# 14chanwa/remotesensingProject

Measured on AMD Instinct MI355X. Metric: Mpixel*disparity-hypotheses/s, higher is better.
Workload: dtype f32

## Files before the change

remotesensingproject_amd/build.py:

```python
from __future__ import annotations

import os
import re
import subprocess
import sys

HERE = os.path.dirname(os.path.abspath(__file__))
CSRC = os.path.join(HERE, "csrc")
OBJ = os.path.join(CSRC, "build")
SO = os.path.join(CSRC, "librslf_hip.so")
INCLUDE = os.path.join(os.path.dirname(HERE), "include")
COMMON = ["rslf_internal.hpp", "rslf_plan.hpp", "rslf_scratch.hpp", "rslf_device.hpp", "k2_taps.hpp", os.path.join(INCLUDE, "rslf_hip.h")]
UNITS = {
    "rslf_core.hip": ["k0_pack.hpp"],
    "rslf_pile.hip": ["k1_edge.hpp", "k_compact.hpp", "k2_scan.hpp", "k2_reg.hpp", "k2_stream.hpp", "k3_median.hpp"],
    "rslf_chip_a.hip": ["k2_scan.hpp", "k2_chip.hpp"],
    "rslf_chip_b.hip": ["k2_scan.hpp", "k2_chip.hpp"],
    "rslf_chip_c.hip": ["k2_scan.hpp", "k2_chip.hpp"],
    "rslf_scores.hip": ["k2_scan.hpp", "k2_reg.hpp", "k2_scores.hpp"],
    "rslf_peaks.hip": ["k8_peaks.hpp", "k8_peak_rule.hpp", "rslf_plan_peaks.hpp"],
    "rslf_subgrid.hip": ["k2_scan.hpp", "k9_subgrid.hpp", "k8_peak_rule.hpp", "rslf_plan_subgrid.hpp"],
    "rslf_sweep.hip": ["k3_median.hpp", "k4_propagate.hpp", "k_compact.hpp", "k2_scan.hpp", "k7_line_conf.hpp", "rslf_plan_subgrid.hpp",
                       "rslf_plan_sweep_peaks.hpp", "rslf_plan_peaks.hpp", "rslf_plan_sweep_gate.hpp", "k11_f2c_peak_rule.hpp"],
    "rslf_sweep_peaks.hip": ["k2_scan.hpp", "k10_sweep_peaks.hpp", "k10_peak_merge.hpp", "k8_peak_rule.hpp", "rslf_plan_sweep_peaks.hpp",
                             "rslf_plan_peaks.hpp", "rslf_plan_subgrid.hpp"],
    "rslf_f2c.hip": ["k5_f2c.hpp", "rslf_plan_f2c_peaks.hpp", "rslf_plan_peaks.hpp", "rslf_plan_f2c_consistency.hpp",
                     "rslf_plan_consistency.hpp", "k12_consistency_rule.hpp"],
    "rslf_f2c_keep.hip": ["rslf_plan_f2c_peaks.hpp", "rslf_plan_peaks.hpp", "rslf_plan_sweep_gate.hpp", "k11_f2c_peak_rule.hpp",
                          "rslf_plan_f2c_consistency.hpp", "rslf_plan_consistency.hpp", "k12_consistency_rule.hpp"],
    "rslf_f2c_peaks.hip": ["k11_f2c_peaks.hpp", "k11_f2c_peak_rule.hpp", "rslf_plan_f2c_peaks.hpp", "rslf_plan_peaks.hpp"],
    "rslf_render.hip": ["k6_render.hpp", "rslf_plan_render.hpp"],
    "rslf_consistency.hip": ["k12_consistency.hpp", "k12_consistency_rule.hpp", "rslf_plan_consistency.hpp", "k13_f2c_consistency.hpp",
                             "rslf_plan_f2c_consistency.hpp"],
    "rslf_warp.hip": ["k14_view_warp.hpp", "k14_warp_rule.hpp", "rslf_plan_warp.hpp", "k12_consistency_rule.hpp"],
    "rslf_multi.hip": [],
    "rslf_multi_sweep.hip": [],
}
SOURCES = list(UNITS)

HIPCC_FLAGS = [
    "--offload-arch=gfx950",
    "-O3",
    "-std=c++17",
    "-fPIC",
    "-ffp-contract=off",
    "-fno-fast-math",
    "-fno-slp-vectorize",
]


def _hipcc() -> str:
    for c in (os.environ.get("HIPCC"), "/opt/rocm/bin/hipcc", "hipcc"):
        if c and (os.path.isabs(c) and os.path.exists(c) or not os.path.isabs(c)):
            return c
    raise RuntimeError("hipcc not found")


def _deps(unit: str) -> list[str]:
    out = []
    for d in [unit] + UNITS[unit] + COMMON:
        p = d if os.path.isabs(d) else os.path.join(CSRC, d)
        if os.path.exists(p):
            out.append(p)
    return out


def _obj(unit: str) -> str:
    return os.path.join(OBJ, unit.replace(".hip", ".o"))


def _stale(unit: str) -> bool:
    o = _obj(unit)
    return not os.path.exists(o) or any(os.path.getmtime(d) > os.path.getmtime(o) for d in _deps(unit))


def needs_build() -> bool:
    return not os.path.exists(SO) or any(_stale(u) or os.path.getmtime(_obj(u)) > os.path.getmtime(SO) for u in SOURCES)


def source_hash() -> str:
    import hashlib
    h = hashlib.sha256()
    files = sorted(set(p for u in SOURCES for p in _deps(u)))
    for p in files:
        h.update(os.path.basename(p).encode() + b"\0")
        h.update(open(p, "rb").read())
    return h.hexdigest()[:16]


def build_variant(name: str, defines: list[str]) -> str:
    import concurrent.futures
    out_dir = os.path.join(os.path.dirname(HERE), "ab")
    os.makedirs(out_dir, exist_ok=True)
    os.makedirs(OBJ, exist_ok=True)

    def compile_unit(u: str) -> str:
        obj = os.path.join(OBJ, "%s_%s.o" % (os.path.splitext(u)[0], name))
        r = subprocess.run([_hipcc()] + HIPCC_FLAGS + ["-D" + d for d in defines] + ["-I", INCLUDE, "-c", u, "-o", obj],
                           cwd=CSRC, capture_output=True, text=True)
        if r.returncode != 0:
            raise RuntimeError("hipcc failed on %s:\n%s" % (u, r.stderr[-4000:]))
        return obj

    with concurrent.futures.ThreadPoolExecutor(max_workers=min(len(SOURCES), os.cpu_count() or 1)) as ex:
        objs = list(ex.map(compile_unit, SOURCES))
    so = os.path.join(out_dir, "librslf_%s.so" % name)
# ... 66 lines not shown
```

remotesensingproject_amd/csrc/k4_propagate.hpp:

```cpp
#pragma once

#include "k_compact.hpp"
#include "k11_f2c_peak_rule.hpp"
#include "k3_median.hpp"
#include "rslf_device.hpp"

#ifndef RSLF_CLAIM_BATCH
#define RSLF_CLAIM_BATCH 8
#endif

namespace rslf {

constexpr int kClaimMaxViews = 1024;
constexpr int kNoWinner = 0x7F7F7F7F;

template <int C>
__device__ __forceinline__ void propagate_claim_pixel(const VolView& vol, int s_hat, int v, int u, float cur, bool source,
                                                      const float* __restrict__ rbar_vu, const uint8_t* __restrict__ mask_svu,
                                                      int* __restrict__ winner_svu, uint8_t* __restrict__ dirty, float slope,
                                                      const plan::NormThreshold& prop_thr, const unsigned long long* live_views)
{
    const int nseg = (vol.U + 255) >> 8;
    const long long o = (long long)v * vol.U + u;
    float rb[C];
#pragma unroll
    for (int c = 0; c < C; c++)
        rb[c] = source ? rbar_vu[o * C + c] : 0.0f;
    const long long plane = (long long)vol.V * vol.U;
    const long long row = (long long)v * vol.U;
    constexpr int B = RSLF_CLAIM_BATCH;
    for (int s0 = 0; s0 < vol.S; s0 += B) {
        int ri[B];
        bool live[B];
        static_assert(64 % B == 0, "a batch of views sits in one word of the live-view bits");
        if (live_views && ((live_views[s0 >> 6] >> (s0 & 63)) & ((1ull << B) - 1ull)) == 0)
            continue;
        uint8_t mb[B];
#pragma unroll
        for (int j = 0; j < B; j++) {
            const int s = s0 + j;
            float off = cur * (float)(s_hat - s);
            off = off * slope;
            ri[j] = u + (int)roundf(off);
            live[j] = source && s < vol.S && ri[j] >= 0 && ri[j] < vol.U;
            ri[j] = min(max(ri[j], 0), vol.U - 1);
            mb[j] = mask_svu[(long long)min(s, vol.S - 1) * plane + row + ri[j]];
        }
        bool any = false;
#pragma unroll
        for (int j = 0; j < B; j++) {
            live[j] = live[j] && mb[j] != 0;
            any |= live[j];
        }
        if (!__any(any))
            continue;
        float e[B][C];
#pragma unroll
        for (int j = 0; j < B; j++) {
            const float* er = vol.row(v, min(s0 + j, vol.S - 1));
            const int col = live[j] ? ri[j] : min(u, vol.U - 1);
#pragma unroll
            for (int c = 0; c < C; c++)
                e[j][c] = er[col * C + c];
        }
#pragma unroll
        for (int j = 0; j < B; j++) {
            if (!live[j])
                continue;
            float df[C];
#pragma unroll
            for (int c = 0; c < C; c++)
                df[c] = e[j][c] - rb[c];
            if (norm_below<C>(df, prop_thr)) {
                atomicMin(&winner_svu[(long long)(s0 + j) * plane + row + ri[j]], u);
                dirty[((long long)(s0 + j) * vol.V + v) * nseg + (ri[j] >> 8)] = 1;
            }
        }
    }
}

struct ClaimGate {
    const int32_t* idx;
    const float* score;
    const int32_t* runner_idx;
    const float* runner_score;
    long long hat;
    float ratio;
    unsigned long long* withheld;
// ... 93 lines not shown
                                                       uint8_t* __restrict__ dirty, float slope, plan::NormThreshold prop_thr,
                                                       const float* __restrict__ gate_Cd_vu, float disp_thr, int* __restrict__ reset,
                                                       const int* __restrict__ remain)
{
    median_claim_body<C, MODE, false>(vol, s_hat, raw_vu, filtered_vu, edge_mask_vu, w, median_thr, rbar_vu, mask_svu, winner_svu, dirty,
                                      slope, prop_thr, gate_Cd_vu, disp_thr, reset, remain, ClaimGate{});
}

template <int C, int MODE>
__global__ __launch_bounds__(256) void k34_median_claim_gated(VolView vol, int s_hat, const float* __restrict__ raw_vu,
                                                             float* __restrict__ filtered_vu, const uint8_t* __restrict__ edge_mask_vu,
                                                             int w, plan::NormThreshold median_thr, const float* __restrict__ rbar_vu,
                                                             const uint8_t* __restrict__ mask_svu, int* __restrict__ winner_svu,
                                                             uint8_t* __restrict__ dirty, float slope, plan::NormThreshold prop_thr,
                                                             const float* __restrict__ gate_Cd_vu, float disp_thr,
                                                             int* __restrict__ reset, const int* __restrict__ remain, ClaimGate gate)
{
    median_claim_body<C, MODE, true>(vol, s_hat, raw_vu, filtered_vu, edge_mask_vu, w, median_thr, rbar_vu, mask_svu, winner_svu, dirty,
                                     slope, prop_thr, gate_Cd_vu, disp_thr, reset, remain, gate);
}

struct ApplyPeaks {
    int32_t* idx;
    float* score;
    int32_t* runner_idx;
    float* runner_score;
};

template <bool PEAKS>
__device__ __forceinline__ void apply_segment(long long r, int seg, int V, int U, const float* __restrict__ filtered_vu,
                                              const float* __restrict__ Cd_hat_vu, float* __restrict__ depth_svu,
                                              float* __restrict__ Cd_svu, uint8_t* mask_svu, int* __restrict__ winner_svu,
                                              int* __restrict__ remain, const float* __restrict__ Cl_hat_vu,
                                              float* __restrict__ Cl_svu, const ApplyPeaks& pk, long long hat)
{
    const int u = (seg << 8) + threadIdx.x;
    const long long t = r * U + (u < U ? u : U - 1);
    const int w = u < U ? winner_svu[t] : U;
    const unsigned long long leaving = __ballot(w < U);
    if (remain && leaving && (threadIdx.x & 63) == 0)
        atomicSub(&remain[r * ((U + 255) >> 8) + seg], __popcll(leaving));
    if (w >= U)
        return;
    const long long src = (r % V) * U + w;
    depth_svu[t] = filtered_vu[src];
    Cd_svu[t] = Cd_hat_vu[src];
    if (Cl_svu)
        Cl_svu[t] = Cl_hat_vu[src];
    if (PEAKS) {
        if (pk.idx)
            pk.idx[t] = pk.idx[hat + src];
        if (pk.score)
            pk.score[t] = pk.score[hat + src];
        if (pk.runner_idx)
            pk.runner_idx[t] = pk.runner_idx[hat + src];
        if (pk.runner_score)
            pk.runner_score[t] = pk.runner_score[hat + src];
    }
    mask_svu[t] = 0;
    winner_svu[t] = kNoWinner;
}

__global__ __launch_bounds__(256) void k4_count_segments(const uint8_t* __restrict__ mask_svu, long long rows, int U, int* __restrict__ remain)
{
    const int nseg = (U + 255) >> 8;
    const long long item = blockIdx.x;
    if (item >= rows * nseg)
        return;
    const long long r = item / nseg;
    const int seg = (int)(item - r * nseg);
    const int u = (seg << 8) + threadIdx.x;
    const unsigned long long b = __ballot(u < U && mask_svu[r * U + (u < U ? u : 0)] != 0);
    __shared__ int s_n[4];
    if ((threadIdx.x & 63) == 0)
        s_n[threadIdx.x >> 6] = __popcll(b);
    __syncthreads();
    if (threadIdx.x == 0)
        remain[item] = s_n[0] + s_n[1] + s_n[2] + s_n[3];
}

constexpr int kApplyRowsPerBlock = 4;
constexpr int kApplyFlagSlots = 1024;

template <bool PEAKS>
__device__ __forceinline__ void propagate_apply_body(int S, int V, int U, int s_hat, const float* __restrict__ filtered_vu,
                                                         const float* __restrict__ Cd_hat_vu, float* __restrict__ depth_svu,
                                                         float* __restrict__ Cd_svu, uint8_t* mask_svu, int* __restrict__ winner_svu,
                                                         uint8_t* __restrict__ dirty, int s_next, const uint8_t* __restrict__ edge_mask_next_vu,
                                                         int* __restrict__ list, int* __restrict__ count,
                                                         unsigned long long* __restrict__ total, int* __restrict__ packed_n,
                                                         int* __restrict__ remain, int* __restrict__ rowbase,
                                                         const float* __restrict__ Cl_hat_vu, float* __restrict__ Cl_svu, const ApplyPeaks& pk)
{
    __shared__ uint8_t s_flags[kApplyFlagSlots];
    const long long hat = PEAKS ? (long long)s_hat * V * U : 0;
    const int nseg = (U + 255) >> 8;
    const int lead = s_next >= 0 ? V : 0;
    if ((int)blockIdx.x < lead) {
        const int v = blockIdx.x;
        const long long r = (long long)s_next * V + v;
        uint8_t* flags = dirty + r * nseg;
        for (int seg = 0; seg < nseg; seg++)
            if (flags[seg])
                apply_segment<PEAKS>(r, seg, V, U, filtered_vu, Cd_hat_vu, depth_svu, Cd_svu, mask_svu, winner_svu, remain, Cl_hat_vu, Cl_svu, pk, hat);
        __syncthreads();
        if ((int)threadIdx.x < nseg)
            flags[threadIdx.x] = 0;
        compact_row_packed(v, edge_mask_next_vu, mask_svu + (long long)s_next * V * U, U, list, count, total, packed_n, rowbase);
        return;
    }
    const long long nrows = (long long)S * V;
    const long long r0 = (long long)(blockIdx.x - lead) * kApplyRowsPerBlock;
    const long long r1 = r0 + kApplyRowsPerBlock < nrows ? r0 + kApplyRowsPerBlock : nrows;
    const int nfl = (int)(r1 - r0) * nseg;
    for (int i = threadIdx.x; i < nfl; i += 256) {
        const long long r = r0 + i / nseg;
        uint8_t f = 0;
        if ((int)(r / V) != s_next) {
            f = dirty[r0 * nseg + i];
            if (f)
                dirty[r0 * nseg + i] = 0;
        }
        s_flags[i] = f;
    }
    __syncthreads();
    for (int i = 0; i < nfl; i++)
        if (s_flags[i])
            apply_segment<PEAKS>(r0 + i / nseg, i % nseg, V, U, filtered_vu, Cd_hat_vu, depth_svu, Cd_svu, mask_svu, winner_svu, remain, Cl_hat_vu, Cl_svu, pk, hat);
}

__global__ __launch_bounds__(256) void k4_propagate_apply(int S, int V, int U, int s_hat, const float* __restrict__ filtered_vu,
                                                         const float* __restrict__ Cd_hat_vu, float* __restrict__ depth_svu,
                                                         float* __restrict__ Cd_svu, uint8_t* mask_svu, int* __restrict__ winner_svu,
                                                         uint8_t* __restrict__ dirty, int s_next, const uint8_t* __restrict__ edge_mask_next_vu,
                                                         int* __restrict__ list, int* __restrict__ count,
                                                         unsigned long long* __restrict__ total, int* __restrict__ packed_n,
                                                         int* __restrict__ remain, int* __restrict__ rowbase,
                                                         const float* __restrict__ Cl_hat_vu, float* __restrict__ Cl_svu)
{
    propagate_apply_body<false>(S, V, U, s_hat, filtered_vu, Cd_hat_vu, depth_svu, Cd_svu, mask_svu, winner_svu, dirty, s_next,
                                edge_mask_next_vu, list, count, total, packed_n, remain, rowbase, Cl_hat_vu, Cl_svu, ApplyPeaks{});
}

__global__ __launch_bounds__(256) void k4_propagate_apply_peaks(int S, int V, int U, int s_hat, const float* __restrict__ filtered_vu,
                                                               const float* __restrict__ Cd_hat_vu, float* __restrict__ depth_svu,
                                                               float* __restrict__ Cd_svu, uint8_t* mask_svu, int* __restrict__ winner_svu,
                                                               uint8_t* __restrict__ dirty, int s_next,
                                                               const uint8_t* __restrict__ edge_mask_next_vu, int* __restrict__ list,
                                                               int* __restrict__ count, unsigned long long* __restrict__ total,
                                                               int* __restrict__ packed_n, int* __restrict__ remain, int* __restrict__ rowbase,
                                                               const float* __restrict__ Cl_hat_vu, float* __restrict__ Cl_svu, ApplyPeaks pk)
{
    propagate_apply_body<true>(S, V, U, s_hat, filtered_vu, Cd_hat_vu, depth_svu, Cd_svu, mask_svu, winner_svu, dirty, s_next,
                               edge_mask_next_vu, list, count, total, packed_n, remain, rowbase, Cl_hat_vu, Cl_svu, pk);
}

}
```

remotesensingproject_amd/csrc/rslf_core.hip:

```cpp
#include "rslf_internal.hpp"

#include <algorithm>
#include <cmath>

#include "k0_pack.hpp"

using namespace rslf;


namespace rslf {

char* last_error_buffer()
{
    static thread_local char g_err[512] = "";
    return g_err;
}

static std::atomic<int> g_inject[kInjectSites];

bool inject_hit(InjectSite site)
{
    std::atomic<int>& c = g_inject[site];
    int v = c.load(std::memory_order_relaxed);
    while (v > 0)
// ... 138 lines not shown
{
    if (!out)
        return fail(RSLF_ERR_INVALID_ARG, "out is NULL");
    *out = nullptr;
    int n = 0;
    if (hipGetDeviceCount(&n) != hipSuccess || n <= 0)
        return fail(RSLF_ERR_NO_DEVICE, "no HIP device visible");
    if (device < 0 || device >= n)
        return fail(RSLF_ERR_INVALID_ARG, "device %d out of range (0..%d)", device, n - 1);
    hipDeviceProp_t prop;
    HIP_TRY(hipGetDeviceProperties(&prop, device));
    if (strncmp(prop.gcnArchName, "gfx950", 6) != 0)
        return fail(RSLF_ERR_NO_DEVICE, "device %d is %s; this library holds gfx950 code objects only", device, prop.gcnArchName);
    HIP_TRY(hipSetDevice(device));
    rslf_ctx* ctx = new (std::nothrow) rslf_ctx();
    if (!ctx)
        return fail(RSLF_ERR_ALLOC, "out of host memory");
    ctx->device = device;
    (void)hipDeviceGetAttribute(&ctx->num_cus, hipDeviceAttributeMultiprocessorCount, device);
    hipError_t e = hip_err(ctx->scratch.total.reserve(2 * sizeof(unsigned long long)));
    if (e == hipSuccess)
        e = hip_err(ctx->scratch.minmax.reserve(2 * sizeof(float)));
    if (e == hipSuccess)
        e = hipEventCreate(&ctx->ev0);
    if (e == hipSuccess)
        e = hipEventCreate(&ctx->ev1);
    if (e != hipSuccess) {
        (void)rslf_ctx_destroy(ctx);
        return fail(RSLF_ERR_HIP, "context setup failed: %s", hipGetErrorString(e));
    }
    *out = ctx;
    return RSLF_OK;
}
RSLF_API_CATCH

extern "C" int rslf_ctx_destroy(rslf_ctx* ctx) RSLF_API_TRY
{
    if (!ctx)
        return RSLF_OK;
    (void)hipSetDevice(ctx->device);
    (void)hipStreamSynchronize(ctx->stream);
    for (hipEvent_t e : ctx->ev_pool)
        (void)hipEventDestroy(e);
    if (ctx->ev0)
        (void)hipEventDestroy(ctx->ev0);
    if (ctx->ev1)
        (void)hipEventDestroy(ctx->ev1);
    delete ctx;
    return RSLF_OK;
}
RSLF_API_CATCH

extern "C" int rslf_ctx_set_stream(rslf_ctx* ctx, void* hip_stream) RSLF_API_TRY
{
    if (!ctx)
        return fail(RSLF_ERR_INVALID_ARG, "ctx is NULL");
    ctx->stream = (hipStream_t)hip_stream;
    return RSLF_OK;
}
RSLF_API_CATCH

extern "C" int rslf_ctx_set_debug(rslf_ctx* ctx, const char* key, int value) RSLF_API_TRY
{
    if (!ctx || !key)
        return fail(RSLF_ERR_INVALID_ARG, "ctx/key is NULL");
    if (strcmp(key, "force_scan") == 0 && value >= 0 && value <= 2)
        ctx->force_scan = value;
    else if (strcmp(key, "force_groups") == 0 && value >= 0 && value <= 64)
        ctx->force_groups = value;
    else if (strcmp(key, "force_packed") == 0 && value >= -1 && value <= 1)
        ctx->force_packed = value;
    else if (strcmp(key, "px") == 0 && value >= -1 && value <= 1)
        ctx->px_mode = value;
    else if (strcmp(key, "stream_share") == 0 && value >= 0 && value <= 2)
        ctx->stream_share = value;
    else if (strcmp(key, "row_split") == 0 && value >= 0 && value <= 65536)
        ctx->row_split = value;
    else if (strcmp(key, "tap_table") == 0 && (value == 0 || value == 1))
        ctx->tap_table = value;
    else if (strcmp(key, "scalar_taps") == 0 && (value == 0 || value == 1))
        ctx->scalar_taps = value;
    else if (strcmp(key, "claim_skip") == 0 && (value == 0 || value == 1))
        ctx->claim_skip = value;
    else if (strcmp(key, "subgrid_list") == 0 && (value == 0 || value == 1))
        ctx->subgrid_list = value;
    else if (strcmp(key, "peaks_list") == 0 && (value == 0 || value == 1))
        ctx->peaks_list = value;
    else if (strcmp(key, "consistency_order") == 0 && value >= 0 && value <= 2)
        ctx->consistency_order = value;
    else if (strcmp(key, "time_all") == 0 && (value == 0 || value == 1)) {
        ctx->time_all = value;
        ctx->ev_used = 0;
    } else if (strcmp(key, "stream_groups") == 0 && value >= 0 && value <= 64)
        ctx->stream_groups = value;
    else if (strcmp(key, "stream_lds_kib") == 0 && value >= 16 && value <= 152) {
        ctx->stream_lds_bytes = (size_t)value << 10;
    } else if (strcmp(key, "staging_kib") == 0 && value >= 0 && value <= 262144)
        ctx->staging_kib = value;
    else
        return fail(RSLF_ERR_INVALID_ARG, "rslf_ctx_set_debug: unknown key or value out of range: %s = %d", key, value);
    return RSLF_OK;
}
RSLF_API_CATCH

extern "C" int rslf_ctx_synchronize(rslf_ctx* ctx) RSLF_API_TRY
{
    if (!ctx)
        return fail(RSLF_ERR_INVALID_ARG, "ctx is NULL");
    HIP_TRY(hipSetDevice(ctx->device));
    HIP_TRY(hipStreamSynchronize(ctx->stream));
    return RSLF_OK;
}
RSLF_API_CATCH


extern "C" int rslf_volume_create(rslf_ctx* ctx, int V, int S, int U, int C, rslf_volume** out) RSLF_API_TRY
{
    if (!ctx || !out)
        return fail(RSLF_ERR_INVALID_ARG, "ctx/out is NULL");
    *out = nullptr;
    if (V < 1 || S < 1 || U < 1)
        return fail(RSLF_ERR_INVALID_ARG, "bad dimensions V=%d S=%d U=%d", V, S, U);
    if (C != 1 && C != 3)
        return fail(RSLF_ERR_UNSUPPORTED, "C=%d: the reference instantiates float and cv::Vec3f only (dc.hpp:149-154)", C);
    if (V > 65535 || S > 65535)
        return fail(RSLF_ERR_UNSUPPORTED, "V=%d / S=%d: the per-scanline kernels index scanlines and views with grid.y / grid.z "
                                          "(at most 65535)", V, S);
    if ((long long)S * C * (((long long)U + 1 + 63) / 64 * 64) > ((long long)1 << 29))
        return fail(RSLF_ERR_UNSUPPORTED, "one EPI (S*pitch*C floats) must stay below 2 GiB: the scan addresses it with 32-bit byte offsets");
    HIP_TRY(hipSetDevice(ctx->device));
    rslf_volume* vol = new (std::nothrow) rslf_volume();
    if (!vol)
        return fail(RSLF_ERR_ALLOC, "out of host memory");
    vol->ctx = ctx;
    vol->device = ctx->device;
    vol->V = V;
    vol->S = S;
    vol->U = U;
    vol->C = C;
    vol->pitch = plan::volume_pitch(U);
    vol->bytes = plan::volume_bytes(V, S, U, C);
    hipError_t e = hipMalloc(&vol->base, vol->bytes);
    if (e != hipSuccess) {
        delete vol;
        return fail(RSLF_ERR_ALLOC, "hipMalloc(%zu) for the volume failed: %s", vol->bytes, hipGetErrorString(e));
    }
    *out = vol;
    return RSLF_OK;
}
RSLF_API_CATCH

extern "C" int rslf_volume_destroy(rslf_volume* vol) RSLF_API_TRY
{
    if (!vol)
        return RSLF_OK;
    (void)hipSetDevice(vol->device);
    (void)hipFree(vol->base);
    delete vol;
    return RSLF_OK;
}
RSLF_API_CATCH

extern "C" int rslf_volume_describe(const rslf_volume* vol, rslf_volume_desc* out) RSLF_API_TRY
{
    if (!vol || !out)
        return fail(RSLF_ERR_INVALID_ARG, "vol/out is NULL");
// ... 428 lines not shown
```

remotesensingproject_amd/csrc/rslf_internal.hpp:

```cpp
#pragma once

#include "../../include/rslf_hip.h"

#include <hip/hip_runtime.h>

#include <atomic>
#include <cstdarg>
#include <cstdio>
#include <cstring>
#include <exception>
#include <functional>
#include <memory>
#include <new>
#include <string>
#include <thread>
#include <vector>

#include "rslf_device.hpp"
#include "rslf_plan.hpp"
#include "rslf_scratch.hpp"


namespace rslf {

// ... 146 lines not shown
    DeviceBuf withheld;
    DeviceBuf lc_columns;
    DeviceBuf lc_argmax;
    DeviceBuf shared[kSharedBufs];

    static constexpr size_t kMaxPartials = 2048;
    unsigned long long* pixel_total() const { return total.as<unsigned long long>(); }
    int* packed_len() const { return reinterpret_cast<int*>(pixel_total() + 1); }
    uint8_t* morph_tmp() const { return depth_tmp.as<uint8_t>(); }
};

constexpr int row_exact_slots(int spad, int C) { return (C == 1 && spad == 104) ? spad : 0; }
constexpr size_t row_exact_bytes(int dim_d, int slots) { return (size_t)dim_d * ((size_t)slots * 16 + 8); }

struct RowExactKey {
    float dmin = 0.0f, dmax = 0.0f, slope = 0.0f;
    int dim_d = 0, s_hat = 0, S = 0, U = 0, C = 0, slots = 0;
    long long stride_s = 0;
    const void* queued_on = nullptr;
    bool same(const RowExactKey& o) const
    {
        return memcmp(&dmin, &o.dmin, sizeof(float)) == 0 && memcmp(&dmax, &o.dmax, sizeof(float)) == 0 &&
               memcmp(&slope, &o.slope, sizeof(float)) == 0 && dim_d == o.dim_d && s_hat == o.s_hat && S == o.S && U == o.U && C == o.C &&
               slots == o.slots && stride_s == o.stride_s && queued_on == o.queued_on;
    }
};

struct SweepState {
    bool open = false;
    bool keep_total = false;
    bool first = true;
    bool scanned = false;
    bool listed = false;
    int expect = -1;
    uint8_t* mask_run = nullptr;
    int lc_mode = RSLF_LINE_CONF_OFF;
    float* lc_Cl_svu = nullptr;
    float* lc_K_vsu = nullptr;
    int32_t* lc_idx_vu = nullptr;
    const float* lc_Ce_svu = nullptr;
    const float* lc_dmin_vu = nullptr;
    const float* lc_dmax_vu = nullptr;
    float lc_dmin = 0.0f, lc_dmax = 0.0f;
    int lc_dim_d = 0;
    ScanConsts lc_consts = {};
    bool subgrid = false;
    bool peaks = false;
    rslf_peaks pk = {};
    int dim_d = 0;
    float prop_ratio = 0.0f;
};

}

struct rslf_ctx {
    int device = 0;
    hipStream_t stream = nullptr;
    rslf::Scratch scratch;
    rslf::SweepState sweep;
    hipEvent_t ev0 = nullptr, ev1 = nullptr;
    bool ev_valid = false;
    int time_all = 0;
    std::vector<hipEvent_t> ev_pool;
    size_t ev_used = 0;
    int last_spad = 0;
    int last_kernel = 0;
    bool last_gated = false;
    int num_cus = 0;
    int force_scan = 0;
    int force_groups = 0;
    int force_packed = -1;
    int px_mode = -1;
    int stream_groups = 0;
    int stream_share = 1;
    size_t stream_lds_bytes = rslf::plan::kStreamLdsBytes;
    int row_split = 1;
    int tap_table = 1;
    int scalar_taps = 1;
    rslf::RowExactKey row_exact_key;
    bool last_row_exact = false;
    int subgrid_list = 1;
    int peaks_list = 1;
    int claim_skip = 1;
    int staging_kib = 0;
    int consistency_order = 0;
};

struct rslf_volume {
    rslf_ctx* ctx = nullptr;
    int device = 0;
    int V = 0, S = 0, U = 0, C = 0, pitch = 0;
    float* base = nullptr;
    size_t bytes = 0;
    float min_value = 0.0f, max_value = 0.0f;
    bool filled = false;
};

struct rslf_multi {
    struct Dev {
        rslf_ctx* ctx = nullptr;
        hipStream_t s_up = nullptr, s_comp = nullptr, s_down = nullptr;
        hipEvent_t done[2] = {nullptr, nullptr};
        rslf_volume* vol[2] = {nullptr, nullptr};
        rslf::DeviceBuf planes[2];
        rslf::PinnedBuf pin[2];
        rslf::DeviceBuf arena;
    };
    std::vector<Dev> devs;
    int chunk_rows = 0;
    std::vector<unsigned char> peer;
};

namespace rslf {

struct StreamScope {
    StreamScope(rslf_ctx* ctx_, hipStream_t stream) : ctx(ctx_), saved(ctx_->stream) { ctx->stream = stream; }
    ~StreamScope() { ctx->stream = saved; }
    StreamScope(const StreamScope&) = delete;
    StreamScope& operator=(const StreamScope&) = delete;
    rslf_ctx* const ctx;
    const hipStream_t saved;
};

inline VolView view_of(const rslf_volume* vol)
{
    VolView w;
    w.base = vol->base;
    w.V = vol->V;
    w.S = vol->S;
    w.U = vol->U;
    w.C = vol->C;
    w.pitch = vol->pitch;
    w.stride_s = (long long)vol->pitch * vol->C;
    w.stride_v = (long long)vol->S * w.stride_s;
    return w;
}

inline float scale_of(float epi_scale_factor)
{
    return (float)(1.0 / (double)epi_scale_factor);
}

struct DevBuf : DeviceBuf {
    hipError_t alloc(size_t bytes) { return hip_err(reserve(bytes ? bytes : 1)); }
};

int check_params(const rslf_params* p);
ScanConsts make_scan_consts(const rslf_params* p);
int ensure_plane_scratch(rslf_ctx* ctx, int V, int U);
int ensure_group_scratch(rslf_ctx* ctx, size_t recs, size_t tiles, bool* tickets_fresh = nullptr);
int ensure_staging(rslf_ctx* ctx, size_t bytes);
int helper_scratch(rslf_ctx* ctx, SharedBuf which, size_t bytes, void** out);
enum class Elem { F32, U8, U16 };
inline size_t elem_bytes(Elem e) { return e == Elem::F32 ? sizeof(float) : e == Elem::U8 ? 1 : sizeof(uint16_t); }
template <typename T>
float host_max(const T* const* h_ptrs, int n_ptrs, int rows, size_t row_stride_bytes, size_t row_elems, float start);
template <typename T>
float host_max_parallel(const T* const* h_epis, int V, int S, size_t stride, size_t row_elems, float start);
float resolve_scale_factor(Elem e, const void* const* h_ptrs, int n_ptrs, int rows, size_t row_stride_bytes, size_t row_elems,
                           float epi_scale_factor, bool parallel);
template <typename SrcT>
int upload_host(rslf_volume* vol, const SrcT* const* h_ptrs, size_t row_stride_bytes, bool image_major, float scale);
extern template int upload_host<float>(rslf_volume*, const float* const*, size_t, bool, float);
extern template int upload_host<uint8_t>(rslf_volume*, const uint8_t* const*, size_t, bool, float);
extern template int upload_host<uint16_t>(rslf_volume*, const uint16_t* const*, size_t, bool, float);
int upload_host_elem(rslf_volume* vol, Elem e, const void* const* h_ptrs, size_t row_stride_bytes, bool image_major, float scale);
// ... 128 lines not shown
```

remotesensingproject_amd/csrc/rslf_sweep.hip:

```cpp
#include "rslf_internal.hpp"
#include "rslf_plan_subgrid.hpp"
#include "rslf_plan_sweep_gate.hpp"
#include "rslf_plan_sweep_peaks.hpp"

#include <algorithm>
#include <cmath>

#include "k3_median.hpp"
#include "k4_propagate.hpp"
#include "k7_line_conf.hpp"

using namespace rslf;


static int ensure_sweep_scratch(rslf_ctx* ctx, const rslf_volume* vol)
{
    Scratch& sc = ctx->scratch;
    const size_t n = (size_t)vol->S * vol->V * vol->U;
    const Reserved w = sc.winner.reserve(n * sizeof(int));
    HIP_TRY(hip_err(w));
    if (w.fresh)
        HIP_TRY(hipMemsetAsync(sc.winner.get(), 0x7F, sc.winner.capacity(), ctx->stream));
    HIP_TRY(hip_err(sc.sweep_mask.reserve(n)));
    const size_t flags = (size_t)vol->S * vol->V * ((vol->U + 255) / 256);
    HIP_TRY(hip_err(sc.remain.reserve(flags * sizeof(int))));
    const Reserved d = sc.dirty.reserve(flags);
    HIP_TRY(hip_err(d));
    if (d.fresh)
        HIP_TRY(hipMemsetAsync(sc.dirty.get(), 0, sc.dirty.capacity(), ctx->stream));
    HIP_TRY(hip_err(sc.filtered.reserve((size_t)vol->V * vol->U * sizeof(float))));
    return RSLF_OK;
}

static void sweep_close(rslf_ctx* ctx, bool ok)
{
    ctx->last_gated = ok && ctx->sweep.prop_ratio > 0.0f;
    ctx->sweep = SweepState();
    if (!ok) {
        ctx->scratch.winner.mark_stale();
        ctx->scratch.dirty.mark_stale();
    }
}

static ScanInputs visit_inputs(bool first, bool listed)
{
    ScanInputs in;
    in.zero_total = false;
    in.timed = first;
    if (!first) {
        in.groups = plan::kSweepGroups;
        in.packed = true;
        in.lists = listed ? ScanInputs::kPackedList : ScanInputs::kCompact;
        in.packed_n_zero = !listed;
    }
    return in;
}

extern "C" int rslf_sweep_begin(rslf_ctx* ctx, const rslf_volume* vol, const uint8_t* d_Ce_mask_svu, uint8_t* d_scan_mask_svu,
                                int dim_d, int v_lo, int v_hi) RSLF_API_TRY
{
    if (!ctx || !vol || !d_Ce_mask_svu)
        return fail(RSLF_ERR_INVALID_ARG, "NULL argument");
    if (v_lo < 0 || v_hi > vol->V || v_lo >= v_hi)
        return fail(RSLF_ERR_INVALID_ARG, "active scanlines [%d, %d) outside the volume's %d", v_lo, v_hi, vol->V);
    HIP_TRY(hipSetDevice(ctx->device));
    if (ctx->sweep.open)
        sweep_close(ctx, false);
    int rc = ensure_sweep_scratch(ctx, vol);
    if (rc)
        return rc;
    const int S = vol->S, V = vol->V, U = vol->U;
    const size_t n = (size_t)V * U;
    hipStream_t st = ctx->stream;
    uint8_t* mask_svu = d_scan_mask_svu ? d_scan_mask_svu : ctx->scratch.sweep_mask.as<uint8_t>();
    HIP_TRY(hipMemcpyAsync(mask_svu, d_Ce_mask_svu, (size_t)S * n, hipMemcpyDeviceToDevice, st));
    if (v_lo > 0)
        HIP_TRY(hipMemset2DAsync(mask_svu, n, 0, (size_t)v_lo * U, S, st));
    if (v_hi < V)
        HIP_TRY(hipMemset2DAsync(mask_svu + (size_t)v_hi * U, n, 0, (size_t)(V - v_hi) * U, S, st));
    HIP_TRY(hipMemsetAsync(ctx->scratch.pixel_total(), 0, sizeof(unsigned long long), st));
    {
        const long long rows = (long long)S * V;
        const long long items = rows * ((U + 255) / 256);
// ... 245 lines not shown
    if (ctx->force_packed == 0 || n > (size_t)INT32_MAX)
        s_next = -1;
    const int lc_mode = ctx->sweep.lc_mode;
    float* Cl = lc_mode ? ctx->sweep.lc_Cl_svu + (size_t)s_hat * n : nullptr;
    auto line_confidence = [&]() -> int {
        LineConfArgs q = {};
        q.V = V, q.S = S, q.U = U, q.s_hat = s_hat;
        q.Ce_svu = ctx->sweep.lc_Ce_svu;
        q.K_vsu = ctx->sweep.lc_K_vsu;
        q.depth_vu = filtered;
        q.mask_vu = cem;
        q.Cl_vu = Cl;
        ScanArgs a = {};
        a.vol = view_of(vol);
        a.dmin_vu = ctx->sweep.lc_dmin_vu, a.dmax_vu = ctx->sweep.lc_dmax_vu;
        a.dmin = ctx->sweep.lc_dmin, a.dmax = ctx->sweep.lc_dmax;
        a.dim_d = ctx->sweep.lc_dim_d;
        a.s_hat = s_hat;
        a.k = ctx->sweep.lc_consts;
        a.groups = 1;
        return launch_line_confidence(ctx, q, a, ctx->sweep.lc_idx_vu, C);
    };
    const plan::SweepGate gate = plan::sweep_gate(p->use_disp_confidence_score != 0, lc_mode);
    const bool k7_first = plan::line_conf_before_claims(p->use_disp_confidence_score != 0, lc_mode);
    bool launched = false;
    if (k7_first) {
#define RSLF_K3_CASE(CC, MODE)                                                                                                    \
    if (!launched && C == CC && mp.mode == MODE) {                                                                                \
        if (mp.lds_bytes > ((size_t)64 << 10))                                                                                    \
            HIP_TRY(hipFuncSetAttribute(reinterpret_cast<const void*>(&k3_selective_median<CC, MODE>),                           \
                                        hipFuncAttributeMaxDynamicSharedMemorySize, (int)mp.lds_bytes));                         \
        hipLaunchKernelGGL((k3_selective_median<CC, MODE>), grid_vu, dim3(kMedianBlock), mp.lds_bytes, st, view_of(vol), depth,   \
                           filtered, cem, s_hat, mp.w, median_thr);                                                               \
        launched = true;                                                                                                          \
    }
        RSLF_MEDIAN_MODES(RSLF_K3_CASE, 1)
        RSLF_MEDIAN_MODES(RSLF_K3_CASE, 3)
#undef RSLF_K3_CASE
        if (!launched)
            return fail(RSLF_ERR_INTERNAL, "no selective-median kernel for %d channels, mode %d", C, mp.mode);
        HIP_TRY(hipGetLastError());
        if (int rc = line_confidence())
            return rc;
        launched = false;
    }
    const float* gate_vu = gate == plan::kGateDispConf ? Cd : gate == plan::kGateLineConf ? Cl : nullptr;
    const float gate_thr = gate == plan::kGateLineConf ? p->line_score_threshold : p->disp_score_threshold;
    const bool gated = ctx->sweep.prop_ratio > 0.0f;
    const ClaimGate cg = {ctx->sweep.pk.idx, ctx->sweep.pk.score, ctx->sweep.pk.runner_idx, ctx->sweep.pk.runner_score,
                          (long long)s_hat * (long long)n, ctx->sweep.prop_ratio, sc.withheld.as<unsigned long long>()};
#define RSLF_K34G_CASE(CC, MODE)                                                                                                 \
    if (gated && !launched && C == CC && mp.mode == MODE) {                                                                       \
        if (mp.lds_bytes > ((size_t)64 << 10))                                                                                    \
            HIP_TRY(hipFuncSetAttribute(reinterpret_cast<const void*>(&k34_median_claim_gated<CC, MODE>),                        \
                                        hipFuncAttributeMaxDynamicSharedMemorySize, (int)mp.lds_bytes));                         \
        hipLaunchKernelGGL((k34_median_claim_gated<CC, MODE>), grid_vu, dim3(256), mp.lds_bytes, st, view_of(vol), s_hat, depth,  \
                           filtered, cem, mp.w, median_thr, rbar, mask_svu, winner, dirty, p->slope_factor, prop_thr,             \
                           gate_vu, gate_thr, packed_n, ctx->claim_skip ? remain : nullptr, cg);                                  \
        launched = true;                                                                                                          \
    }
    RSLF_MEDIAN_MODES(RSLF_K34G_CASE, 1)
    RSLF_MEDIAN_MODES(RSLF_K34G_CASE, 3)
#undef RSLF_K34G_CASE
#define RSLF_K34_CASE(CC, MODE)                                                                                                  \
    if (!launched && C == CC && mp.mode == MODE) {                                                                                \
        if (mp.lds_bytes > ((size_t)64 << 10))                                                                                    \
            HIP_TRY(hipFuncSetAttribute(reinterpret_cast<const void*>(&k34_median_claim<CC, MODE>),                              \
                                        hipFuncAttributeMaxDynamicSharedMemorySize, (int)mp.lds_bytes));                         \
        hipLaunchKernelGGL((k34_median_claim<CC, MODE>), grid_vu, dim3(256), mp.lds_bytes, st, view_of(vol), s_hat, depth, filtered, \
                           cem, mp.w, median_thr, rbar, mask_svu, winner, dirty, p->slope_factor, prop_thr,                       \
                           gate_vu, gate_thr, packed_n,                                                                           \
                           ctx->claim_skip ? remain : nullptr);                                                                   \
        launched = true;                                                                                                          \
    }
    RSLF_MEDIAN_MODES(RSLF_K34_CASE, 1)
    RSLF_MEDIAN_MODES(RSLF_K34_CASE, 3)
#undef RSLF_K34_CASE
    if (!launched)
        return fail(RSLF_ERR_INTERNAL, "no median + claims kernel for %d channels, mode %d", C, mp.mode);
    HIP_TRY(hipGetLastError());
    if (lc_mode != RSLF_LINE_CONF_OFF && !k7_first)
        if (int rc = line_confidence())
            return rc;
    const unsigned apply_blocks = (unsigned)((s_next >= 0 ? V : 0) + ((long long)S * V + kApplyRowsPerBlock - 1) / kApplyRowsPerBlock);
    const uint8_t* const next_mask = s_next >= 0 ? d_Ce_mask_svu + (size_t)s_next * n : nullptr;
    float* const Cl_svu = lc_mode ? ctx->sweep.lc_Cl_svu : nullptr;
    if (ctx->sweep.peaks) {
        const rslf_peaks& pk = ctx->sweep.pk;
        const ApplyPeaks apk = {pk.idx, pk.score, pk.runner_idx, pk.runner_score};
        hipLaunchKernelGGL(k4_propagate_apply_peaks, dim3(apply_blocks), dim3(256), 0, st, S, V, U, s_hat, filtered, Cd, d_depth_svu,
                           d_Cd_svu, mask_svu, winner, dirty, s_next, next_mask, sc.list.as<int>(), sc.count.as<int>(),
                           sc.pixel_total(), packed_n, remain, sc.rowbase.as<int>(), Cl, Cl_svu, apk);
    } else {
        hipLaunchKernelGGL(k4_propagate_apply, dim3(apply_blocks), dim3(256), 0, st, S, V, U, s_hat, filtered, Cd, d_depth_svu,
                           d_Cd_svu, mask_svu, winner, dirty, s_next, next_mask, sc.list.as<int>(), sc.count.as<int>(),
                           sc.pixel_total(), packed_n, remain, sc.rowbase.as<int>(), Cl, Cl_svu);
    }
    HIP_TRY(hipGetLastError());
    ctx->sweep.listed = s_next >= 0;
    ctx->sweep.expect = s_after;
    ctx->sweep.first = false;
    return RSLF_OK;
}
RSLF_API_CATCH

extern "C" int rslf_sweep_end(rslf_ctx* ctx, int ok, int dim_d, rslf_stats* stats) RSLF_API_TRY
{
    if (!ctx)
        return fail(RSLF_ERR_INVALID_ARG, "ctx is NULL");
    const bool was_open = ctx->sweep.open;
    sweep_close(ctx, ok != 0 && was_open);
    if (ok && was_open && stats) {
        HIP_TRY(hipSetDevice(ctx->device));
        return read_stats(ctx, dim_d, stats);
    }
    return RSLF_OK;
}
RSLF_API_CATCH

static int entry_gate_check(float ratio, const rslf_peaks* pk)
{
    return gate_refusal(plan::sweep_gate_entry_args(ratio, pk != nullptr, pk && pk->idx, pk && pk->score, pk && pk->runner_idx,
                                                    pk && pk->runner_score),
                        ratio, "the sweep");
}

static int depth_epi_2d(rslf_ctx* ctx, const rslf_volume* vol, const float* d_dmin_svu, const float* d_dmax_svu, float dmin,
                        float dmax, int dim_d, float* d_Ce_svu, uint8_t* d_Ce_mask_svu, float* d_Cd_svu, float* d_depth_svu,
                        float* d_rbar_svu, const rslf_params* p, uint8_t* d_scan_mask_svu, rslf_stats* stats, int line_mode,
                        float* d_Cl_svu, int subgrid, const rslf_peaks* d_pk_svu = nullptr, float propagation_ratio = 0.0f)
{
    if (!ctx || !vol || !d_Ce_svu || !d_Ce_mask_svu || !d_Cd_svu || !d_depth_svu || !d_rbar_svu)
        return fail(RSLF_ERR_INVALID_ARG, "NULL argument");
    if (int rc = entry_gate_check(propagation_ratio, d_pk_svu))
        return rc;
    if (!plan::line_conf_mode_ok(line_mode))
        return fail(RSLF_ERR_INVALID_ARG, "line confidence mode %d: must be RSLF_LINE_CONF_OFF, _AS_BUILT or _GATE", line_mode);
    if (line_mode != RSLF_LINE_CONF_OFF && !d_Cl_svu)
        return fail(RSLF_ERR_INVALID_ARG, "line confidence mode %d needs the [S][V][U] plane", line_mode);
    if (subgrid != 0 && subgrid != 1)
        return fail(RSLF_ERR_INVALID_ARG, "subgrid=%d: 0 or 1", subgrid);
    int rc = check_params(p);
    if (rc)
        return rc;
    rc = rslf_sweep_begin(ctx, vol, d_Ce_mask_svu, d_scan_mask_svu, dim_d, 0, vol->V);
    if (rc)
        return rc;
    if (line_mode != RSLF_LINE_CONF_OFF)
        rc = rslf_sweep_line_confidence(ctx, vol, line_mode, d_Cl_svu);
    if (!rc && subgrid)
        rc = rslf_sweep_subgrid(ctx, vol, 1);
    if (!rc && d_pk_svu)
        rc = rslf_sweep_peaks(ctx, vol, d_pk_svu);
    if (!rc && propagation_ratio != 0.0f)
        rc = rslf_sweep_propagation_ratio(ctx, vol, propagation_ratio);
    for (int s_hat : plan::sweep_order(vol->S)) {
        if (!rc)
            rc = rslf_sweep_visit_scan(ctx, vol, d_dmin_svu, d_dmax_svu, dmin, dmax, dim_d, s_hat, d_Ce_svu, d_Ce_mask_svu, d_Cd_svu,
                                       d_depth_svu, d_rbar_svu, p);
        if (!rc)
            rc = rslf_sweep_visit_finish(ctx, vol, s_hat, d_Ce_mask_svu, d_Cd_svu, d_depth_svu, d_rbar_svu, p);
        if (rc) {
            const std::string msg = last_error_buffer();
            (void)rslf_sweep_end(ctx, 0, dim_d, nullptr);
            return fail(rc, "%s", msg.c_str());
        }
    }
    return rslf_sweep_end(ctx, 1, dim_d, stats);
}

extern "C" int rslf_depth_epi_2d(rslf_ctx* ctx, const rslf_volume* vol, const float* d_dmin_svu, const float* d_dmax_svu,
                                 float dmin, float dmax, int dim_d, float* d_Ce_svu, uint8_t* d_Ce_mask_svu, float* d_Cd_svu,
                                 float* d_depth_svu, float* d_rbar_svu, const rslf_params* p, uint8_t* d_scan_mask_svu,
                                 rslf_stats* stats) RSLF_API_TRY
{
    return depth_epi_2d(ctx, vol, d_dmin_svu, d_dmax_svu, dmin, dmax, dim_d, d_Ce_svu, d_Ce_mask_svu, d_Cd_svu, d_depth_svu, d_rbar_svu,
                        p, d_scan_mask_svu, stats, RSLF_LINE_CONF_OFF, nullptr, 0);
}
RSLF_API_CATCH
// ... 240 lines not shown
```

remotesensingproject_amd/depth.py:

```python
from __future__ import annotations

import atexit
import copy
import ctypes as C
import sys
from dataclasses import dataclass
from typing import NamedTuple, Optional, Sequence

import numpy as np
import torch

from . import _lib
from ._lib import RslfParams, RslfStats, RslfVolumeDesc, check


class Interpolation1DLinear:
    mode = 0


class Interpolation1DNearestNeighbour:

    def __init__(self, as_built: bool = False):
        self.mode = 2 if as_built else 1

# ... 19 lines not shown
    par_interpolation_class: object = 0
    par_use_disp_confidence_score: bool = False
    par_line_confidence_mode: int = 0

    @staticmethod
    def get_default() -> "Depth1DParameters":
        return Depth1DParameters()

    def to_c(self) -> RslfParams:
        p = RslfParams()
        for f, _ in RslfParams._fields_:
            if f == "interpolation":
                p.interpolation = int(getattr(self.par_interpolation_class, "mode", self.par_interpolation_class))
                continue
            v = getattr(self, "par_" + f)
            setattr(p, f, int(v) if isinstance(getattr(p, f), int) else float(v))
        return p


LINE_CONF_OFF, LINE_CONF_AS_BUILT, LINE_CONF_GATE = 0, 1, 2


def require_no_line_confidence(parameters, who: str) -> None:
    if parameters is not None and int(parameters.par_line_confidence_mode) != LINE_CONF_OFF:
        raise ValueError("%s: par_line_confidence_mode=%d is not built here (one-device Depth2DComputer only)"
                         % (who, int(parameters.par_line_confidence_mode)))


def require_no_subgrid(subgrid, who: str) -> None:
    if subgrid:
        raise ValueError("%s: subgrid=True is not built here (one device: Depth1DComputer_pile, Depth1DComputer, "
                         "Depth2DComputer, FineToCoarse, fine_to_coarse_run_host and the compute_*_depth_epi functions)" % who)


def require_no_peaks(peaks, who: str) -> None:
    if peaks is not None and peaks is not False:
        raise ValueError("%s: peaks is not built here (one device, one sweep: Depth2DComputer and compute_2D_depth_epi)" % who)


def _ratio_on(ratio) -> bool:
    return ratio is not None and ratio is not False and ratio != 0


def require_no_propagation_ratio(ratio, who: str) -> None:
    if _ratio_on(ratio):
        raise ValueError("%s: propagation_ratio is not built here (one device, a sweep in the peaks mode: Depth2DComputer, "
                         "compute_2D_depth_epi and fine_to_coarse_run_host(keep=True, peaks=True))" % who)


def require_no_consistency_gate(min_agree, who: str) -> None:
    if min_agree is not None and min_agree is not False and min_agree != 0:
        raise ValueError("%s: consistency_min_agree is not built here (one device, a kept run: fine_to_coarse_run_host(keep=True))" % who)


def _propagation_ratio(ratio, who: str) -> float:
    if not _ratio_on(ratio):
        return 0.0
    r = float(ratio)
    if not 0.0 < r <= 1.0:
        raise ValueError("%s: propagation_ratio %r is not in (0, 1]" % (who, ratio))
    return r


class Context:

    def __init__(self, device: int | torch.device | None = None):
        if device is None:
            device = torch.cuda.current_device()
        self.device = torch.device("cuda", device) if isinstance(device, int) else torch.device(device)
        h = C.c_void_p()
        check(_lib.lib().rslf_ctx_create(self.device.index or 0, C.byref(h)), "rslf_ctx_create")
        self._h = h
        self.use_current_stream()

    def use_current_stream(self) -> None:
        s = torch.cuda.current_stream(self.device).cuda_stream
        check(_lib.lib().rslf_ctx_set_stream(self._h, C.c_void_p(s)), "rslf_ctx_set_stream")

    def synchronize(self) -> None:
        check(_lib.lib().rslf_ctx_synchronize(self._h), "rslf_ctx_synchronize")

    _DEBUG_DEFAULTS = dict(force_scan=0, force_groups=0, force_packed=-1, px=-1, stream_share=1, stream_groups=0, stream_lds_kib=80,
                           claim_skip=1, time_all=0, row_split=1, staging_kib=0, tap_table=1, scalar_taps=1,
                           subgrid_list=1, peaks_list=1, consistency_order=0)
    _FORCE_SCAN = {None: 0, "auto": 0, "generic": 1, "stream": 2}

    def set_debug(self, **hooks) -> None:
        for k, v in hooks.items():
            if k == "force_scan" and not isinstance(v, int):
                v = self._FORCE_SCAN[v or None]
            check(_lib.lib().rslf_ctx_set_debug(self._h, k.encode(), int(v)), "rslf_ctx_set_debug(%s)" % k)

    def reset_debug(self) -> None:
        self.set_debug(**self._DEBUG_DEFAULTS)

    def last_scan_kernel_ms(self) -> float:
        ms = C.c_float()
        check(_lib.lib().rslf_last_scan_kernel_ms(self._h, C.byref(ms)), "rslf_last_scan_kernel_ms")
        return float(ms.value)

    def last_scan_row_exact(self) -> tuple[bool, int]:
        a, n = C.c_int(), C.c_int()
        check(_lib.lib().rslf_last_scan_row_exact(self._h, C.byref(a), C.byref(n)), "rslf_last_scan_row_exact")
        return bool(a.value), int(n.value)

    def scan_time_total_ms(self) -> tuple[float, int]:
        ms, n = C.c_float(), C.c_int()
        check(_lib.lib().rslf_scan_time_total_ms(self._h, C.byref(ms), C.byref(n)), "rslf_scan_time_total_ms")
        return float(ms.value), int(n.value)

    def get_withheld_sources(self) -> int:
        n = C.c_ulonglong()
        check(_lib.lib().rslf_sweep_withheld(self._h, C.byref(n)), "rslf_sweep_withheld")
        return int(n.value)

    def close(self) -> None:
        if getattr(self, "_h", None) and not sys.is_finalizing():
            _lib.lib().rslf_ctx_destroy(self._h)
        self._h = None

    def __del__(self):
        try:
            self.close()
        except Exception:
            pass


_DEFAULT_CTX: dict[int, Context] = {}


@atexit.register
def _drop_default_contexts() -> None:
    for c in list(_DEFAULT_CTX.values()):
        c._h = None
    _DEFAULT_CTX.clear()


def default_context(device=None) -> Context:
    idx = torch.cuda.current_device() if device is None else torch.device(device).index or 0
    if idx not in _DEFAULT_CTX:
        _DEFAULT_CTX[idx] = Context(idx)
    return _DEFAULT_CTX[idx]


def _ptr(t: Optional[torch.Tensor]) -> C.c_void_p:
    return C.c_void_p(0 if t is None else t.data_ptr())


_SUFFIX = {np.dtype(np.uint8): "u8", np.dtype(np.uint16): "u16", np.dtype(np.float32): "f32"}


def field_dtype(dtype) -> np.dtype:
    dt = np.dtype(dtype)
    return dt if dt in (np.uint8, np.uint16) else np.dtype(np.float32)


class Volume:

    def __init__(self, ctx: Context, V: int, S: int, U: int, C_: int):
        self.ctx = ctx
        h = C.c_void_p()
        check(_lib.lib().rslf_volume_create(ctx._h, V, S, U, C_, C.byref(h)), "rslf_volume_create")
        self._h = h
        self.V, self.S, self.U, self.C = V, S, U, C_
        self.scale_used: float | None = None

    @staticmethod
# ... 1649 lines not shown
```

Measured before the change: 8482.

## Use a fixed-size strided grid for sparse propagate-apply after first sweep step

Replaces the apply kernel's one-block-per-four-rows grid with a fixed grid capped at a multiple of the CU count, where each block strides over dirty segment flags, ballots the dirty ones into shared memory and processes them. This is on by default for every sweep step after the first. The aim is to avoid launching and retiring many blocks that find few dirty segments when the dirty set is sparse. In exchange, the work per block becomes less balanced and each step of the loop adds barriers.

```diff
diff --git a/remotesensingproject_amd/build.py b/remotesensingproject_amd/build.py
--- a/remotesensingproject_amd/build.py
+++ b/remotesensingproject_amd/build.py
@@ -21,7 +21,8 @@
     "rslf_peaks.hip": ["k8_peaks.hpp", "k8_peak_rule.hpp", "rslf_plan_peaks.hpp"],
     "rslf_subgrid.hip": ["k2_scan.hpp", "k9_subgrid.hpp", "k8_peak_rule.hpp", "rslf_plan_subgrid.hpp"],
     "rslf_sweep.hip": ["k3_median.hpp", "k4_propagate.hpp", "k_compact.hpp", "k2_scan.hpp", "k7_line_conf.hpp", "rslf_plan_subgrid.hpp",
-                       "rslf_plan_sweep_peaks.hpp", "rslf_plan_peaks.hpp", "rslf_plan_sweep_gate.hpp", "k11_f2c_peak_rule.hpp"],
+                       "rslf_plan_sweep_peaks.hpp", "rslf_plan_peaks.hpp", "rslf_plan_sweep_gate.hpp", "k11_f2c_peak_rule.hpp",
+                       "rslf_plan_sparse_grids.hpp"],
     "rslf_sweep_peaks.hip": ["k2_scan.hpp", "k10_sweep_peaks.hpp", "k10_peak_merge.hpp", "k8_peak_rule.hpp", "rslf_plan_sweep_peaks.hpp",
                              "rslf_plan_peaks.hpp", "rslf_plan_subgrid.hpp"],
     "rslf_f2c.hip": ["k5_f2c.hpp", "rslf_plan_f2c_peaks.hpp", "rslf_plan_peaks.hpp", "rslf_plan_f2c_consistency.hpp",
diff --git a/remotesensingproject_amd/csrc/k4_propagate.hpp b/remotesensingproject_amd/csrc/k4_propagate.hpp
--- a/remotesensingproject_amd/csrc/k4_propagate.hpp
+++ b/remotesensingproject_amd/csrc/k4_propagate.hpp
@@ -4,6 +4,7 @@
 #include "k11_f2c_peak_rule.hpp"
 #include "k3_median.hpp"
 #include "rslf_device.hpp"
+#include "rslf_plan_sparse_grids.hpp"
 
 #ifndef RSLF_CLAIM_BATCH
 #define RSLF_CLAIM_BATCH 8
@@ -263,7 +264,7 @@
 constexpr int kApplyRowsPerBlock = 4;
 constexpr int kApplyFlagSlots = 1024;
 
-template <bool PEAKS>
+template <bool PEAKS, bool FIXED>
 __device__ __forceinline__ void propagate_apply_body(int S, int V, int U, int s_hat, const float* __restrict__ filtered_vu,
                                                          const float* __restrict__ Cd_hat_vu, float* __restrict__ depth_svu,
                                                          float* __restrict__ Cd_svu, uint8_t* mask_svu, int* __restrict__ winner_svu,
@@ -290,6 +291,33 @@
         compact_row_packed(v, edge_mask_next_vu, mask_svu + (long long)s_next * V * U, U, list, count, total, packed_n, rowbase);
         return;
     }
+    if (FIXED) {
+        static_assert(plan::kApplyStepFlags == 256, "one flag byte per thread, one 64-bit word of the queue per wave");
+        __shared__ unsigned long long s_queue[4];
+        const long long nflags = (long long)S * V * nseg;
+        const long long G = gridDim.x - lead, g = blockIdx.x - lead;
+        for (long long base = 0; plan::apply_flag_of(g, G, base) < nflags; base += plan::kApplyStepFlags) {
+            const long long i = plan::apply_flag_of(g, G, base + threadIdx.x);
+            bool mine = false;
+            if (i < nflags && plan::apply_flag_general(i, nseg, V, s_next)) {
+                mine = dirty[i] != 0;
+                if (mine)
+                    dirty[i] = 0;
+            }
+            const unsigned long long b = __ballot(mine);
+            if ((threadIdx.x & 63) == 0)
+                s_queue[threadIdx.x >> 6] = b;
+            __syncthreads();
+            for (int w = 0; w < 4; w++)
+                for (unsigned long long m = s_queue[w]; m != 0; m &= m - 1) {
+                    const long long f = plan::apply_flag_of(g, G, base + w * 64 + (__ffsll(m) - 1));
+                    apply_segment<PEAKS>(plan::apply_flag_row(f, nseg), plan::apply_flag_segment(f, nseg), V, U, filtered_vu, Cd_hat_vu,
+                                         depth_svu, Cd_svu, mask_svu, winner_svu, remain, Cl_hat_vu, Cl_svu, pk, hat);
+                }
+            __syncthreads();
+        }
+        return;
+    }
     const long long nrows = (long long)S * V;
     const long long r0 = (long long)(blockIdx.x - lead) * kApplyRowsPerBlock;
     const long long r1 = r0 + kApplyRowsPerBlock < nrows ? r0 + kApplyRowsPerBlock : nrows;
@@ -310,6 +338,7 @@
             apply_segment<PEAKS>(r0 + i / nseg, i % nseg, V, U, filtered_vu, Cd_hat_vu, depth_svu, Cd_svu, mask_svu, winner_svu, remain, Cl_hat_vu, Cl_svu, pk, hat);
 }
 
+template <bool FIXED>
 __global__ __launch_bounds__(256) void k4_propagate_apply(int S, int V, int U, int s_hat, const float* __restrict__ filtered_vu,
                                                          const float* __restrict__ Cd_hat_vu, float* __restrict__ depth_svu,
                                                          float* __restrict__ Cd_svu, uint8_t* mask_svu, int* __restrict__ winner_svu,
@@ -319,10 +348,11 @@
                                                          int* __restrict__ remain, int* __restrict__ rowbase,
                                                          const float* __restrict__ Cl_hat_vu, float* __restrict__ Cl_svu)
 {
-    propagate_apply_body<false>(S, V, U, s_hat, filtered_vu, Cd_hat_vu, depth_svu, Cd_svu, mask_svu, winner_svu, dirty, s_next,
+    propagate_apply_body<false, FIXED>(S, V, U, s_hat, filtered_vu, Cd_hat_vu, depth_svu, Cd_svu, mask_svu, winner_svu, dirty, s_next,
                                 edge_mask_next_vu, list, count, total, packed_n, remain, rowbase, Cl_hat_vu, Cl_svu, ApplyPeaks{});
 }
 
+template <bool FIXED>
 __global__ __launch_bounds__(256) void k4_propagate_apply_peaks(int S, int V, int U, int s_hat, const float* __restrict__ filtered_vu,
                                                                const float* __restrict__ Cd_hat_vu, float* __restrict__ depth_svu,
                                                                float* __restrict__ Cd_svu, uint8_t* mask_svu, int* __restrict__ winner_svu,
@@ -332,7 +362,7 @@
                                                                int* __restrict__ packed_n, int* __restrict__ remain, int* __restrict__ rowbase,
                                                                const float* __restrict__ Cl_hat_vu, float* __restrict__ Cl_svu, ApplyPeaks pk)
 {
-    propagate_apply_body<true>(S, V, U, s_hat, filtered_vu, Cd_hat_vu, depth_svu, Cd_svu, mask_svu, winner_svu, dirty, s_next,
+    propagate_apply_body<true, FIXED>(S, V, U, s_hat, filtered_vu, Cd_hat_vu, depth_svu, Cd_svu, mask_svu, winner_svu, dirty, s_next,
                                edge_mask_next_vu, list, count, total, packed_n, remain, rowbase, Cl_hat_vu, Cl_svu, pk);
 }
 
diff --git a/remotesensingproject_amd/csrc/rslf_core.hip b/remotesensingproject_amd/csrc/rslf_core.hip
--- a/remotesensingproject_amd/csrc/rslf_core.hip
+++ b/remotesensingproject_amd/csrc/rslf_core.hip
@@ -244,6 +244,8 @@
         ctx->scalar_taps = value;
     else if (strcmp(key, "claim_skip") == 0 && (value == 0 || value == 1))
         ctx->claim_skip = value;
+    else if (strcmp(key, "sparse_grids") == 0 && value >= 0 && value <= 2)
+        ctx->sparse_grids = value;
     else if (strcmp(key, "subgrid_list") == 0 && (value == 0 || value == 1))
         ctx->subgrid_list = value;
     else if (strcmp(key, "peaks_list") == 0 && (value == 0 || value == 1))
diff --git a/remotesensingproject_amd/csrc/rslf_internal.hpp b/remotesensingproject_amd/csrc/rslf_internal.hpp
--- a/remotesensingproject_amd/csrc/rslf_internal.hpp
+++ b/remotesensingproject_amd/csrc/rslf_internal.hpp
@@ -252,6 +252,7 @@
     int subgrid_list = 1;
     int peaks_list = 1;
     int claim_skip = 1;
+    int sparse_grids = 1;
     int staging_kib = 0;
     int consistency_order = 0;
 };
diff --git a/remotesensingproject_amd/csrc/rslf_plan_sparse_grids.hpp b/remotesensingproject_amd/csrc/rslf_plan_sparse_grids.hpp
--- /dev/null
+++ b/remotesensingproject_amd/csrc/rslf_plan_sparse_grids.hpp
@@ -0,0 +1,43 @@
+#pragma once
+
+#include <stddef.h>
+
+#if defined(__HIPCC__)
+#define RSLF_SPARSE_GRID_FN __host__ __device__ __forceinline__
+#else
+#define RSLF_SPARSE_GRID_FN inline
+#endif
+
+namespace rslf {
+namespace plan {
+
+constexpr int kApplyStepFlags = 256;
+constexpr int kApplyBlocksPerCu = 16;
+
+inline bool apply_grid_fixed(int hook, bool first_visit) { return hook == 2 || (hook == 1 && !first_visit); }
+
+constexpr int kApplyMinFlags = 8;
+
+inline unsigned apply_general_blocks(int num_cus, long long flags)
+{
+    if (flags <= 0)
+        return 0;
+    const long long want = (flags + kApplyMinFlags - 1) / kApplyMinFlags;
+    const long long cap = (long long)kApplyBlocksPerCu * (num_cus > 0 ? num_cus : 256);
+    const long long g = want < cap ? want : cap;
+    return (unsigned)(g - (g % 2 == 0));
+}
+
+RSLF_SPARSE_GRID_FN long long apply_flag_of(long long g, long long G, long long k) { return k * G + g; }
+
+RSLF_SPARSE_GRID_FN bool apply_flag_general(long long i, int nseg, int V, int s_next)
+{
+    const long long per_view = (long long)V * nseg;
+    return s_next < 0 || i < s_next * per_view || i >= (s_next + 1) * per_view;
+}
+
+RSLF_SPARSE_GRID_FN long long apply_flag_row(long long i, int nseg) { return i / nseg; }
+RSLF_SPARSE_GRID_FN int apply_flag_segment(long long i, int nseg) { return (int)(i - (i / nseg) * nseg); }
+
+}
+}
diff --git a/remotesensingproject_amd/csrc/rslf_sweep.hip b/remotesensingproject_amd/csrc/rslf_sweep.hip
--- a/remotesensingproject_amd/csrc/rslf_sweep.hip
+++ b/remotesensingproject_amd/csrc/rslf_sweep.hip
@@ -1,4 +1,5 @@
 #include "rslf_internal.hpp"
+#include "rslf_plan_sparse_grids.hpp"
 #include "rslf_plan_subgrid.hpp"
 #include "rslf_plan_sweep_gate.hpp"
 #include "rslf_plan_sweep_peaks.hpp"
@@ -410,19 +411,24 @@
     if (lc_mode != RSLF_LINE_CONF_OFF && !k7_first)
         if (int rc = line_confidence())
             return rc;
-    const unsigned apply_blocks = (unsigned)((s_next >= 0 ? V : 0) + ((long long)S * V + kApplyRowsPerBlock - 1) / kApplyRowsPerBlock);
+    const bool fixed = plan::apply_grid_fixed(ctx->sparse_grids, ctx->sweep.first);
+    const long long nflags = (long long)S * V * ((U + 255) / 256);
+    const unsigned apply_blocks = (unsigned)(s_next >= 0 ? V : 0) +
+                                  (fixed ? plan::apply_general_blocks(ctx->num_cus, nflags)
+                                         : (unsigned)(((long long)S * V + kApplyRowsPerBlock - 1) / kApplyRowsPerBlock));
     const uint8_t* const next_mask = s_next >= 0 ? d_Ce_mask_svu + (size_t)s_next * n : nullptr;
     float* const Cl_svu = lc_mode ? ctx->sweep.lc_Cl_svu : nullptr;
     if (ctx->sweep.peaks) {
         const rslf_peaks& pk = ctx->sweep.pk;
         const ApplyPeaks apk = {pk.idx, pk.score, pk.runner_idx, pk.runner_score};
-        hipLaunchKernelGGL(k4_propagate_apply_peaks, dim3(apply_blocks), dim3(256), 0, st, S, V, U, s_hat, filtered, Cd, d_depth_svu,
-                           d_Cd_svu, mask_svu, winner, dirty, s_next, next_mask, sc.list.as<int>(), sc.count.as<int>(),
-                           sc.pixel_total(), packed_n, remain, sc.rowbase.as<int>(), Cl, Cl_svu, apk);
+        hipLaunchKernelGGL(fixed ? k4_propagate_apply_peaks<true> : k4_propagate_apply_peaks<false>, dim3(apply_blocks), dim3(256), 0, st,
+                           S, V, U, s_hat, filtered, Cd, d_depth_svu, d_Cd_svu, mask_svu, winner, dirty, s_next, next_mask,
+                           sc.list.as<int>(), sc.count.as<int>(), sc.pixel_total(), packed_n, remain, sc.rowbase.as<int>(), Cl, Cl_svu,
+                           apk);
     } else {
-        hipLaunchKernelGGL(k4_propagate_apply, dim3(apply_blocks), dim3(256), 0, st, S, V, U, s_hat, filtered, Cd, d_depth_svu,
-                           d_Cd_svu, mask_svu, winner, dirty, s_next, next_mask, sc.list.as<int>(), sc.count.as<int>(),
-                           sc.pixel_total(), packed_n, remain, sc.rowbase.as<int>(), Cl, Cl_svu);
+        hipLaunchKernelGGL(fixed ? k4_propagate_apply<true> : k4_propagate_apply<false>, dim3(apply_blocks), dim3(256), 0, st, S, V, U,
+                           s_hat, filtered, Cd, d_depth_svu, d_Cd_svu, mask_svu, winner, dirty, s_next, next_mask, sc.list.as<int>(),
+                           sc.count.as<int>(), sc.pixel_total(), packed_n, remain, sc.rowbase.as<int>(), Cl, Cl_svu);
     }
     HIP_TRY(hipGetLastError());
     ctx->sweep.listed = s_next >= 0;
diff --git a/remotesensingproject_amd/depth.py b/remotesensingproject_amd/depth.py
--- a/remotesensingproject_amd/depth.py
+++ b/remotesensingproject_amd/depth.py
@@ -125,7 +125,7 @@
 
     _DEBUG_DEFAULTS = dict(force_scan=0, force_groups=0, force_packed=-1, px=-1, stream_share=1, stream_groups=0, stream_lds_kib=80,
                            claim_skip=1, time_all=0, row_split=1, staging_kib=0, tap_table=1, scalar_taps=1,
-                           subgrid_list=1, peaks_list=1, consistency_order=0)
+                           subgrid_list=1, peaks_list=1, consistency_order=0, sparse_grids=1)
     _FORCE_SCAN = {None: 0, "auto": 0, "generic": 1, "stream": 2}
 
     def set_debug(self, **hooks) -> None:
```

New measurement: 8479. No clear change (-0.0%).
